# daultanigaurav/AI-BASED-FRAME-INTERPOLATION

Measured on AMD Instinct MI355X. Metric: interpolated frames/sec at 1080p, higher is better.
Workload: dtype bf16

## Files before the change

ai_based_frame_interpolation_amd/csrc/conv3x3_mfma.hip.h:

```cpp
#pragma once
#include <hip/hip_runtime.h>
#include <stdint.h>
#include <type_traits>

namespace fiunet {

typedef __attribute__((ext_vector_type(4))) float f32x4;
typedef __attribute__((ext_vector_type(8))) __bf16 bf16x8;
typedef __attribute__((ext_vector_type(8))) _Float16 f16x8;

enum SrcMode { SRC_DIRECT = 0, SRC_POOL = 1 , SRC_CONCAT_UP = 2,
               SRC_STEM = 3 ,
               SRC_DIRECT_X2 = 4,
               SRC_STEM_X2 = 5 };
constexpr bool src_is_stem(int mode) { return mode == SRC_STEM || mode == SRC_STEM_X2; }
constexpr bool src_is_x2(int mode) { return mode == SRC_DIRECT_X2 || mode == SRC_STEM_X2; }

__device__ __forceinline__ size_t blk_off(int plane, int y, int x, int H, int W)
{
    return (((size_t)plane * H + y) * W + x) * 64;
}

struct ConvArgs {
    const void* src0;
// ... 159 lines not shown
                                              float ly)
{
    constexpr int NE = Elem<T>::NE;
    float fa[NE], fb[NE], fc[NE], fd[NE], r[NE];
    chunk_unpack<T>(a, fa); chunk_unpack<T>(b, fb); chunk_unpack<T>(c, fc); chunk_unpack<T>(d, fd);
#pragma unroll
    for (int i = 0; i < NE; ++i) {
        const float top = fmaf(lx, fb[i], __fmul_rn(hx, fa[i]));
        const float bot = fmaf(lx, fd[i], __fmul_rn(hx, fc[i]));
        r[i] = fmaf(ly, bot, __fmul_rn(hy, top));
    }
    return chunk_pack<T>(r);
}

template <typename T>
__device__ __forceinline__ void chunk_hlerp(const uint4& a, const uint4& b, float hx, float lx, float* h)
{
    constexpr int NE = Elem<T>::NE;
    float fa[NE], fb[NE];
    chunk_unpack<T>(a, fa); chunk_unpack<T>(b, fb);
#pragma unroll
    for (int i = 0; i < NE; ++i) h[i] = fmaf(lx, fb[i], __fmul_rn(hx, fa[i]));
}
template <typename T>
__device__ __forceinline__ uint4 chunk_vlerp(const float* top, const float* bot, float hy, float ly)
{
    constexpr int NE = Elem<T>::NE;
    float r[NE];
#pragma unroll
    for (int i = 0; i < NE; ++i) r[i] = fmaf(ly, bot[i], __fmul_rn(hy, top[i]));
    return chunk_pack<T>(r);
}


__device__ __forceinline__ uint4 ldg16(const char* p) { return *reinterpret_cast<const uint4*>(p); }

__device__ __forceinline__ float preprocess_u8_value(unsigned char u)
{
    const float x = (float)u, r = 1.0f / 255.0f;
    const float q0 = __fmul_rn(x, r);
    const float q = fmaf(fmaf(-q0, 255.0f, x), r, q0);
    return __fsub_rn(__fmul_rn(2.0f, q), 1.0f);
}
__device__ __forceinline__ unsigned char postprocess_u8_value(float x)
{
    float v = __fdiv_rn(__fadd_rn(x, 1.0f), 2.0f);
    v = fminf(fmaxf(v, 0.0f), 1.0f);
    return (unsigned char)(int)__fmul_rn(v, 255.0f);
}

__device__ __forceinline__ float stem_dither(int y, int x)
{
    const unsigned a = (unsigned)(x ^ y) & 7u, b = (unsigned)y & 7u;
    const unsigned m = ((a & 1u) << 5) | ((b & 1u) << 4) | ((a & 2u) << 2) | ((b & 2u) << 1) | ((a & 4u) >> 1) | ((b & 4u) >> 2);
    return ((float)m + 0.5f) * (1.0f / 64.0f) - 0.5f;
}

struct UpAxis {
    int i0, i1;
    float h, l;
    bool ok;
};
__device__ __forceinline__ UpAxis up_axis(int c, int off, int pad, int lowNg, float scale, int lowOff,
                                          int lowN)
{
    UpAxis u;
    int cu = c + off - pad;
    u.ok = (cu >= 0) & (cu < 2 * lowNg);
    cu = min(max(cu, 0), 2 * lowNg - 1);
    const float f = scale * (float)cu;
    const int g0 = (int)f;
    const int g1 = g0 < lowNg - 1 ? g0 + 1 : g0;
    u.l = f - (float)g0;
    u.h = 1.0f - u.l;
    u.i0 = min(max(g0 - lowOff, 0), lowN - 1);
    u.i1 = min(max(g1 - lowOff, 0), lowN - 1);
    return u;
}
__device__ __forceinline__ UpAxis up_axis_y(const ConvArgs& a, int y)
{
    return up_axis(y, a.upOffY, a.padT, a.lowHg, a.sy, a.lowOffY, a.lowH);
}
__device__ __forceinline__ UpAxis up_axis_x(const ConvArgs& a, int x)
{
    return up_axis(x, 0, a.padL, a.lowW, a.sx, 0, a.lowW);
}
struct UpCoord {
    int y0, y1, x0, x1;
    float hy, ly, hx, lx;
    bool ok;
};
__device__ __forceinline__ UpCoord up_coord(const ConvArgs& a, int y, int x)
{
    const UpAxis v = up_axis_y(a, y), h = up_axis_x(a, x);
    UpCoord u;
    u.y0 = v.i0; u.y1 = v.i1; u.hy = v.h; u.ly = v.l;
    u.x0 = h.i0; u.x1 = h.i1; u.hx = h.h; u.lx = h.l;
    u.ok = v.ok & h.ok;
    return u;
}

template <typename T, int MODE>
__device__ __forceinline__ uint4 gather_chunk(const ConvArgs& a, int b, int y, int x, int plane,
                                              int ch)
{
    constexpr int PL = Elem<T>::PL;
    bool ok = (y >= 0) & (y < a.H) & (x >= 0) & (x < a.W);
    y = min(max(y, 0), a.H - 1);
    x = min(max(x, 0), a.W - 1);
    const int p0 = a.C0 / PL;
    uint4 v;
    if (MODE == SRC_DIRECT || plane < p0) {
        const char* p = (const char*)a.src0 + (size_t)b * a.H * a.W * a.C0 * sizeof(T) +
                        blk_off(plane, y, x, a.H, a.W) + ch * 16;
        v = ldg16(p);
    } else {
        const UpCoord u = up_coord(a, y, x);
        ok = ok & u.ok;
        const char* base = (const char*)a.src1 + (size_t)b * a.lowH * a.lowW * a.C1 * sizeof(T) + ch * 16;
        const int q = plane - p0;
        const uint4 v00 = ldg16(base + blk_off(q, u.y0, u.x0, a.lowH, a.lowW));
        const uint4 v01 = ldg16(base + blk_off(q, u.y0, u.x1, a.lowH, a.lowW));
        const uint4 v10 = ldg16(base + blk_off(q, u.y1, u.x0, a.lowH, a.lowW));
        const uint4 v11 = ldg16(base + blk_off(q, u.y1, u.x1, a.lowH, a.lowW));
        v = chunk_bilerp<T>(v00, v01, v10, v11, u.hx, u.lx, u.hy, u.ly);
    }
    return ok ? v : make_uint4(0u, 0u, 0u, 0u);
}

__device__ __forceinline__ void glds16(const char* gsrc, unsigned lds_wave_base)
{
    unsigned keep;
    asm volatile("s_mov_b32 %0, m0\n\ts_mov_b32 m0, %2\n\ts_nop 0\n\t"
                 "global_load_lds_dwordx4 %1, off\n\ts_mov_b32 m0, %0"
                 : "=&s"(keep)
                 : "v"(gsrc), "s"(lds_wave_base)
                 : "memory");
}
__device__ __forceinline__ void glds16s(const char* sbase, unsigned voff, unsigned lds_wave_base)
{
    unsigned keep;
    asm volatile("s_mov_b32 %0, m0\n\ts_mov_b32 m0, %3\n\ts_nop 0\n\t"
                 "global_load_lds_dwordx4 %1, %2\n\ts_mov_b32 m0, %0"
                 : "=&s"(keep)
                 : "v"(voff), "s"(sbase), "s"(lds_wave_base)
                 : "memory");
}
__device__ __forceinline__ void lds_dma_wait_all() { asm volatile("s_waitcnt vmcnt(0)" ::: "memory"); }
__device__ __forceinline__ unsigned lds_addr_of(const char* p)
{
    return (unsigned)(uintptr_t)(__attribute__((address_space(3))) const char*)p;
}

__device__ __forceinline__ int swz(int row) { return ((row >> 2) & 1) << 1; }

template <typename T>
__device__ __forceinline__ void mma_chunk(f32x4& acc, const uint4& wa, const uint4& xb);
template <>
__device__ __forceinline__ void mma_chunk<__bf16>(f32x4& acc, const uint4& wa, const uint4& xb)
{
    acc = __builtin_amdgcn_mfma_f32_16x16x32_bf16(__builtin_bit_cast(bf16x8, wa),
                                                  __builtin_bit_cast(bf16x8, xb), acc, 0, 0, 0);
}
template <>
__device__ __forceinline__ void mma_chunk<_Float16>(f32x4& acc, const uint4& wa, const uint4& xb)
{
    acc = __builtin_amdgcn_mfma_f32_16x16x32_f16(__builtin_bit_cast(f16x8, wa),
                                                 __builtin_bit_cast(f16x8, xb), acc, 0, 0, 0);
}
template <>
__device__ __forceinline__ void mma_chunk<float>(f32x4& acc, const uint4& wa, const uint4& xb)
{
    acc = __builtin_amdgcn_mfma_f32_16x16x4f32(__uint_as_float(wa.x), __uint_as_float(xb.x), acc, 0, 0, 0);
    acc = __builtin_amdgcn_mfma_f32_16x16x4f32(__uint_as_float(wa.y), __uint_as_float(xb.y), acc, 0, 0, 0);
    acc = __builtin_amdgcn_mfma_f32_16x16x4f32(__uint_as_float(wa.z), __uint_as_float(xb.z), acc, 0, 0, 0);
    acc = __builtin_amdgcn_mfma_f32_16x16x4f32(__uint_as_float(wa.w), __uint_as_float(xb.w), acc, 0, 0, 0);
}

enum Epilogue { EPI_PLAIN = 0, EPI_HEAD = 1 , EPI_POOL = 2, EPI_HEAD3 = 3 ,
                EPI_SPLITK = 4  };
constexpr bool epi_is_splitk(int epi) { return epi == EPI_SPLITK; }

__device__ __forceinline__ unsigned dpp_swap_pairs(unsigned v)
{
    return (unsigned)__builtin_amdgcn_update_dpp(0, (int)v, 0xB1, 0xF, 0xF, true);
}

constexpr int up_segments(int rows, int ncol)
{
    int best = 1, best_cost = 1 << 30;
    for (int n = 1; n <= 6; ++n) {
        const int passes = (n * ncol + 255) / 256, segr = (rows + n - 1) / n;
        const int cost = passes * (segr * 4 + 3);
        if (cost < best_cost) { best_cost = cost; best = n; }
    }
    return best;
}

template <int BN, int TH, int TW, int MODE> struct ConvTile {
    static constexpr int TWP = ((TW + 2 + 7) / 8) * 8;
    static constexpr int THP = TH + 2;
    static constexpr int IN_BYTES = THP * TWP * 64;
    static constexpr int W_BYTES = 3 * BN * 64;
    static constexpr int LRH = (TH + 1) / 2 + 3, LRW = (TW + 1) / 2 + 3, LRP = ((LRW + 3) / 4) * 4;
    static constexpr int LR_PIECES = (LRH * LRP + 15) / 16;
    static constexpr int SPARE_BYTES =
        (MODE == SRC_CONCAT_UP && LR_PIECES * 1024 > W_BYTES) ? LR_PIECES * 1024 - W_BYTES : 0;
    static constexpr int W_STRIDE = W_BYTES + SPARE_BYTES;
    static constexpr int PATCH_W = TW + 4, PATCH_H = TH + 4, PATCH_PITCH = 2 * PATCH_W;
    static_assert(!src_is_stem(MODE) || (2 * PATCH_PITCH) % 32 == 16, "patch pitch: lane groups 0/1 must not share banks");
    static constexpr int PATCH_OFF = IN_BYTES + 2 * W_BYTES + SPARE_BYTES;
    static constexpr int PATCH_TAIL_OFF = (TW + 2) * 64;
    static constexpr int PATCH_TAIL = 2 * PATCH_W * 4;
    static_assert(!src_is_stem(MODE) || PATCH_TAIL_OFF + PATCH_TAIL <= TWP * 64, "bias operand must fit the row-pitch filler");
    static constexpr int PATCH_BYTES = src_is_stem(MODE) ? PATCH_H * PATCH_PITCH * 4 : 0;
    static constexpr int TAB_OFF = PATCH_OFF + ((PATCH_BYTES + 15) / 16) * 16;
    static constexpr int TAB_BYTES = MODE == SRC_CONCAT_UP ? ((THP + TW + 2) * 16 + 255) / 256 * 256 : 0;
    static constexpr int STEMW_OFF = TAB_OFF + TAB_BYTES;
    static constexpr int STEMW_BYTES = src_is_stem(MODE) ? 4096 : 0;
    static constexpr int LDS_BYTES = STEMW_OFF + STEMW_BYTES;
    static_assert(LDS_BYTES <= 80 * 1024, "two workgroups must fit in the CU's 160 KiB of LDS");
    static_assert(!src_is_stem(MODE) || LDS_BYTES <= 63 * 1280, "fused-stem kernel: stay below 64 LDS granules");
};

constexpr int conv_wave_frags(int BN, int TH, int TW) { return TH * TW / 16 / (4 / (BN / 64)); }
constexpr int conv_occupancy(int BN, int TH, int TW, int lds_bytes = 0)
{
    return conv_wave_frags(BN, TH, TW) == 4 && lds_bytes * 3 <= 160 * 1024 ? 3 : 2;
}


__device__ __forceinline__ int conv_block_remap()
{
    const int nblk = gridDim.x, bid = blockIdx.x;
    const int q = nblk >> 3, r = nblk & 7, xcd = bid & 7;
    return (xcd < r ? xcd * (q + 1) : r * (q + 1) + (xcd - r) * q) + (bid >> 3);
}

struct ConvTileId { int ct, b, ty, tx; };
__device__ __forceinline__ ConvTileId conv_tile_decode(const ConvArgs& a, int t)
{
    ConvTileId d;
    d.ct = t % a.nct; t /= a.nct;
    d.tx = t % a.tilesX; t /= a.tilesX;
    d.ty = t % a.tilesY;
    d.b = t / a.tilesY;
    return d;
}

template <typename T> __device__ __forceinline__ int conv_cout_ofs(int m, int lc)
{
    return sizeof(T) == 2 ? (m >> 1) * 32 + lc * 8 + (m & 1) * 4 : m * 16 + lc * 4;
}

template <typename T, int BN, int TH, int TW, int EPI>
__device__ __forceinline__ void conv_acc_init(const ConvArgs& a, f32x4 (&acc)[4][conv_wave_frags(BN, TH, TW)],
                                              int ct, int wc, int lc)
{
    constexpr int NF = conv_wave_frags(BN, TH, TW);
#pragma unroll
    for (int m = 0; m < 4; ++m) {
        f32x4 v = f32x4{0.f, 0.f, 0.f, 0.f};
        if constexpr (!epi_is_splitk(EPI)) {
            const float4 sh = *reinterpret_cast<const float4*>(a.shift + ct * BN + wc * 64 + conv_cout_ofs<T>(m, lc));
            v = f32x4{sh.x, sh.y, sh.z, sh.w};
        }
#pragma unroll
        for (int n = 0; n < NF; ++n) acc[m][n] = v;
    }
}

__device__ __forceinline__ unsigned relu_pk_bf16(unsigned p) { return pk_max_i16(p, 0u); }
__device__ __forceinline__ void relu_fma(float& sum, float x, float lo, float w)
{
    float t;
    asm("v_max_f32 %1, %3, %2\n\tv_fmac_f32 %0, %1, %4" : "+v"(sum), "=&v"(t) : "v"(x), "v"(lo), "v"(w));
}

template <typename T, int BN, int TH, int TW, int EPI, bool X2 = false>
__device__ __forceinline__ void conv_epilogue(const ConvArgs& a, f32x4 (&acc)[4][conv_wave_frags(BN, TH, TW)],
                                              int b, int y0, int x0, int ct, int split, int wc, int wp,
                                              int l15, int lc)
{
    constexpr int PL = Elem<T>::PL;
    constexpr int FR = TW / 16;
    constexpr int NF = conv_wave_frags(BN, TH, TW);
    constexpr int ROWS_W = NF / FR;
    constexpr int HNC = EPI == EPI_HEAD ? 1 : (EPI == EPI_HEAD3 ? 3 : 0);
    const int aH = a.H, aW = a.W;
    constexpr bool PERM = sizeof(T) == 2;
    const int wbase_c = ct * BN + wc * 64;
    if constexpr (epi_is_splitk(EPI)) {
        const int tile = (((b * a.tilesY) + y0 / TH) * a.tilesX + x0 / TW) * a.nct + ct;
        const int ntile = a.B * a.tilesY * a.tilesX * a.nct;
        const int wave = wp * (BN / 64) + wc;
        float4* o = reinterpret_cast<float4*>(a.kslab) + ((((size_t)split * ntile + tile) * 4 + wave) * (4 * NF)) * 64 + (lc * 16 + l15);
#pragma unroll
        for (int m = 0; m < 4; ++m)
#pragma unroll
            for (int n = 0; n < NF; ++n)
                o[(m * NF + n) * 64] = make_float4(acc[m][n][0], acc[m][n][1], acc[m][n][2], acc[m][n][3]);
        return;
    }
    float hw[HNC > 0 ? HNC : 1][4][4];
#pragma unroll
    for (int c = 0; c < HNC; ++c)
#pragma unroll
        for (int m = 0; m < 4; ++m) {
            const float4 v = *reinterpret_cast<const float4*>(a.head_w + c * 64 + conv_cout_ofs<T>(m, lc));
            hw[c][m][0] = v.x; hw[c][m][1] = v.y; hw[c][m][2] = v.z; hw[c][m][3] = v.w;
        }
    const size_t plane_stride = (size_t)aH * aW * 64;
    const int plane0 = wbase_c / PL;
    const int rec_byte = lc * 16;
    char* const out_img = a.dst ? (char*)a.dst + (size_t)b * plane_stride * (a.Cout / PL) +
                                  (size_t)plane0 * plane_stride + rec_byte : nullptr;
    const int pH = aH >> 1, pW = aW >> 1;
    const size_t pplane_stride = (size_t)pH * pW * 64;
    char* const pool_img = EPI == EPI_POOL ? (char*)a.pool_dst + (size_t)b * pplane_stride * (a.Cout / PL) +
                                             (size_t)plane0 * pplane_stride + rec_byte : nullptr;
    if constexpr (HNC > 0) {
        static_assert(HNC == 0 || NF == 8 || NF == 4, "head reduction is written for 8 or 4 fragments per wave");
        const float floor_v = a.relu ? 0.f : -__builtin_inff();
        float hb[HNC];
#pragma unroll
        for (int c = 0; c < HNC; ++c) hb[c] = a.head_b[c];
        const int nb = ((lc & 1) ? 4 : 0) + ((lc & 2) ? 2 : 0);
#pragma unroll
        for (int c = 0; c < HNC; ++c) {
            float hs[NF];
#pragma unroll
            for (int n = 0; n < NF; ++n) {
                float sum = 0.f;
#pragma unroll
                for (int m = 0; m < 4; ++m)
#pragma unroll
                    for (int j = 0; j < 4; ++j) relu_fma(sum, acc[m][n][j], floor_v, hw[c][m][j]);
                hs[n] = sum;
            }
            if constexpr (NF == 4) {
                float full[NF];
#pragma unroll
                for (int n = 0; n < NF; ++n) {
                    const float p = hs[n] + __shfl_xor(hs[n], 16);
                    full[n] = p + __shfl_xor(p, 32);
                }
                const float mine = lc == 0 ? full[0] : (lc == 1 ? full[1] : (lc == 2 ? full[2] : full[3]));
                const int n = lc;
                const int y = y0 + wp * ROWS_W + n / FR;
                const int x = x0 + (n % FR) * 16 + l15;
                if (y < aH && x < aW) {
                    const size_t o = (size_t)b * a.head_img_stride + ((size_t)c * aH + y) * aW + x;
                    if (a.head_out_u8) a.head_out_u8[o] = postprocess_u8_value(mine + hb[c]);
                    else a.head_out[o] = mine + hb[c];
                }
            } else {
                float t[4], u[2];
#pragma unroll
                for (int i = 0; i < 4; ++i) {
                    const auto r = __builtin_amdgcn_permlane16_swap(__float_as_uint(hs[i]), __float_as_uint(hs[(i + 4) % NF]), false, false);
                    t[i] = __uint_as_float(r[0]) + __uint_as_float(r[1]);
                }
#pragma unroll
                for (int j = 0; j < 2; ++j) {
                    const auto r = __builtin_amdgcn_permlane32_swap(__float_as_uint(t[j]), __float_as_uint(t[j + 2]), false, false);
                    u[j] = __uint_as_float(r[0]) + __uint_as_float(r[1]);
                }
#pragma unroll
                for (int j = 0; j < 2; ++j) {
                    const int n = nb + j;
                    const int y = y0 + wp * ROWS_W + n / FR;
                    const int x = x0 + (n % FR) * 16 + l15;
                    if (y < aH && x < aW) {
// ... 102 lines not shown
                const uint4 t = pk[0][g], u = pk[1][g];
                const unsigned c0 = pk_max_i16(t.x, u.x), c1 = pk_max_i16(t.y, u.y);
                const unsigned c2 = pk_max_i16(t.z, u.z), c3 = pk_max_i16(t.w, u.w);
                const uint4 m = make_uint4(pk_max_i16(c0, dpp_swap_pairs(c0)), pk_max_i16(c1, dpp_swap_pairs(c1)),
                                           pk_max_i16(c2, dpp_swap_pairs(c2)), pk_max_i16(c3, dpp_swap_pairs(c3)));
                if (okp) *reinterpret_cast<uint4*>(o + g * pplane_stride) = m;
            }
        }
        return;
    }
#pragma unroll
    for (int n = 0; n < NF; ++n) {
        const int y = y0 + wp * ROWS_W + n / FR;
        const int x = x0 + (n % FR) * 16 + l15;
        const bool ok = (y < aH) && (x < aW);
        if (ok && out_img) {
            char* o = out_img + (size_t)(y * aW + x) * 64;
            if constexpr (PERM) {
#pragma unroll
                for (int g = 0; g < 2; ++g) {
                    uint4 pk = make_uint4(pack2<T>(acc[2 * g][n][0], acc[2 * g][n][1]),
                                          pack2<T>(acc[2 * g][n][2], acc[2 * g][n][3]),
                                          pack2<T>(acc[2 * g + 1][n][0], acc[2 * g + 1][n][1]),
                                          pack2<T>(acc[2 * g + 1][n][2], acc[2 * g + 1][n][3]));
                    if (a.relu) pk = make_uint4(relu_pk_bf16(pk.x), relu_pk_bf16(pk.y), relu_pk_bf16(pk.z), relu_pk_bf16(pk.w));
                    *reinterpret_cast<uint4*>(o + g * plane_stride) = pk;
                }
            } else {
#pragma unroll
                for (int m = 0; m < 4; ++m) {
                    float4 v = make_float4(acc[m][n][0], acc[m][n][1], acc[m][n][2], acc[m][n][3]);
                    if (a.relu) v = make_float4(fmaxf(v.x, 0.f), fmaxf(v.y, 0.f), fmaxf(v.z, 0.f), fmaxf(v.w, 0.f));
                    *reinterpret_cast<float4*>(o + m * plane_stride) = v;
                }
            }
        }
    }
    if (EPI == EPI_POOL) {
#pragma unroll
        for (int n = 0; n < NF; ++n) {
            if (((n / FR) & 1) != 0) continue;
            const int y = y0 + wp * ROWS_W + n / FR;
            const int x = x0 + (n % FR) * 16 + l15;
            const int py = y >> 1, px = x >> 1;
            const bool okp = (py < pH) && (px < pW) && ((l15 & 1) == 0);
            char* o = pool_img + (size_t)(min(py, pH - 1) * pW + min(px, pW - 1)) * 64;
            if constexpr (!PERM) {
#pragma unroll
                for (int m = 0; m < 4; ++m) {
                    float r[4];
#pragma unroll
                    for (int j = 0; j < 4; ++j) {
                        const float cm = fmaxf(acc[m][n][j], acc[m][n + FR][j]);
                        r[j] = fmaxf(cm, __uint_as_float(dpp_swap_pairs(__float_as_uint(cm))));
                        if (a.relu) r[j] = fmaxf(r[j], 0.f);
                    }
                    if (okp) *reinterpret_cast<float4*>(o + m * pplane_stride) = make_float4(r[0], r[1], r[2], r[3]);
                }
            } else {
#pragma unroll
                for (int g = 0; g < 2; ++g) {
                    unsigned r[4];
#pragma unroll
                    for (int h = 0; h < 2; ++h) {
                        const int m = 2 * g + h;
                        const unsigned a0 = pk_max_i16(pack2_pk<T>(acc[m][n][0], acc[m][n][1]),
                                                       pack2_pk<T>(acc[m][n + FR][0], acc[m][n + FR][1]));
                        const unsigned a1 = pk_max_i16(pack2_pk<T>(acc[m][n][2], acc[m][n][3]),
                                                       pack2_pk<T>(acc[m][n + FR][2], acc[m][n + FR][3]));
                        r[2 * h] = pk_max_i16(a0, dpp_swap_pairs(a0));
                        r[2 * h + 1] = pk_max_i16(a1, dpp_swap_pairs(a1));
                        if (a.relu) { r[2 * h] = relu_pk_bf16(r[2 * h]); r[2 * h + 1] = relu_pk_bf16(r[2 * h + 1]); }
                    }
                    if (okp) *reinterpret_cast<uint4*>(o + g * pplane_stride) = make_uint4(r[0], r[1], r[2], r[3]);
                }
            }
        }
    }
}

template <typename T, int BN, int TH, int TW, int MODE, int EPI>
__global__ __launch_bounds__(256, conv_occupancy(BN, TH, TW, ConvTile<BN, TH, TW, MODE>::LDS_BYTES)) void conv3x3_mfma_kernel(const ConvArgs a)
{
    using Tile = ConvTile<BN, TH, TW, MODE>;
    constexpr int PL = Elem<T>::PL;
    constexpr int TWP = Tile::TWP, THP = Tile::THP;
    constexpr int WAVES_C = BN / 64, WAVES_P = 4 / WAVES_C;
    constexpr int FR = TW / 16;
    constexpr int NF = conv_wave_frags(BN, TH, TW);
    constexpr int ROWS_W = NF / FR;
    static_assert(NF == 8 || NF == 4, "wave tile must be 64 couts x 128 or 64 pixels");
    static_assert(TH == ROWS_W * WAVES_P && ROWS_W * FR == NF, "tile does not split over the waves");
    static_assert(EPI != EPI_POOL || ROWS_W % 2 == 0, "pooled epilogue: a wave owns whole row pairs");
    static_assert(Tile::LDS_BYTES * conv_occupancy(BN, TH, TW, Tile::LDS_BYTES) <= 160 * 1024, "LDS per CU");
    constexpr int HNC = EPI == EPI_HEAD ? 1 : (EPI == EPI_HEAD3 ? 3 : 0);
    static_assert(HNC == 0 || BN == 64, "fused head needs all 64 couts in one wave");
    static_assert(MODE == SRC_DIRECT || MODE == SRC_CONCAT_UP || MODE == SRC_STEM || MODE == SRC_DIRECT_X2 ||
                  MODE == SRC_STEM_X2, "pooling is fused into the producer");
    constexpr bool X2 = src_is_x2(MODE);
    constexpr bool STEM = src_is_stem(MODE);
    constexpr bool DIRECT = MODE == SRC_DIRECT || MODE == SRC_DIRECT_X2;
    static_assert(!X2 || std::is_same_v<T, __bf16>, "two-piece operands are bf16");
    static_assert(!STEM || (sizeof(T) == 2 && BN == 64), "fused stem: 2-byte output (bf16 / fp16), 64 couts");

    extern __shared__ __attribute__((aligned(16))) char smem[];
    char* const lds_in = smem;
    char* const lds_w = smem + Tile::IN_BYTES;
    const unsigned lds_in_addr = lds_addr_of(lds_in);
    const unsigned lds_w_addr = lds_addr_of(lds_w);

    int lid = conv_block_remap();
    const int ksplit = epi_is_splitk(EPI) ? a.ksplit : 1;
    const int split = lid % ksplit;
    lid /= ksplit;
    const ConvTileId id = conv_tile_decode(a, lid);
    const int ct = id.ct, b = id.b;
    const int y0 = id.ty * TH, x0 = id.tx * TW;

    const int tid = threadIdx.x;
    const int lane = tid & 63, wave = __builtin_amdgcn_readfirstlane(tid >> 6);
    const int l15 = lane & 15, lc = lane >> 4;
    const int wc = wave % WAVES_C, wp = wave / WAVES_C;

#ifdef FIUNET_STAMP
    unsigned long long st_sum[16] = {0, 0, 0, 0, 0, 0, 0, 0, 0, 0, 0, 0, 0, 0, 0, 0};
    unsigned long long st_t0 = __builtin_amdgcn_s_memtime(), st_prev = st_t0;
#ifdef FIUNET_STAMP_PROLOG
    unsigned long long st_pprev = st_t0;
#define PSTAMP(slot) do { __builtin_amdgcn_sched_barrier(0); const unsigned long long t_ = __builtin_amdgcn_s_memtime(); \
                          st_sum[slot] += t_ - st_pprev; st_pprev = t_; __builtin_amdgcn_sched_barrier(0); } while (0)
#else
#define PSTAMP(slot) do {} while (0)
#endif
#define STAMP(slot) do { const unsigned long long t_ = __builtin_amdgcn_s_memtime(); \
                         st_sum[slot] += t_ - st_prev; st_prev = t_; } while (0)
#define STAMP_UP(slot) STAMP(slot)
#else
#define STAMP(slot) do {} while (0)
#define STAMP_UP(slot) do {} while (0)
#define PSTAMP(slot) do {} while (0)
#endif
    f32x4 acc[4][NF];
    conv_acc_init<T, BN, TH, TW, EPI>(a, acc, ct, wc, lc);
#ifdef FIUNET_STAMP_PROLOG
    asm volatile("" :: "v"(acc[3][NF - 1][3]), "v"(acc[0][0][0]));
#endif
    PSTAMP(9);

    const int a_off = (wc * 64 + l15) * 64 + ((lc ^ swz(l15)) << 4);
    int b_off[3];
#pragma unroll
    for (int kx = 0; kx < 3; ++kx)
        b_off[kx] = (wp * ROWS_W * TWP + kx + l15) * 64 + ((lc ^ swz(kx + l15)) << 4);

    const int nplanes_real = (a.C0 + a.C1) / PL;
    const int nplanes_all = X2 ? 3 * nplanes_real : nplanes_real;
    const int p0 = a.C0 / PL;
    const int pbeg = split * nplanes_all / ksplit, pend = (split + 1) * nplanes_all / ksplit;
    const int nsteps = (pend - pbeg) * 3;
    const char* wbase = (const char*)a.wgt + (size_t)ct * BN * 64;

    constexpr int NW = Tile::W_BYTES / 1024 / 4;
    static_assert(BN % 16 == 0, "a weight piece must not straddle two taps");
    const unsigned w_lane_off = (unsigned)((lane >> 2) * 64 + (((lane & 3) ^ swz(lane >> 2)) << 4));
    auto issue_w = [&](int step) __attribute__((always_inline)) {
        const int lp = step / 3, kx = step - lp * 3;
        int pl = pbeg + lp;
        if constexpr (X2) {
            const int real = pl / 3;
            pl = pl - real * 3 == 1 ? nplanes_real + real : real;
        }
        const char* wsrc = wbase + ((size_t)(pl * 9 + kx * 3) * a.Cout) * 64;
        const unsigned dst = __builtin_amdgcn_readfirstlane(
            lds_w_addr + (unsigned)((step & 1) * Tile::W_STRIDE + wave * NW * 1024));
#pragma unroll
        for (int j = 0; j < NW; ++j) {
            const int r0 = (wave * NW + j) * 16, tap = r0 / BN;
            glds16s(wsrc + (size_t)(tap * (a.Cout - BN) + r0) * 64, w_lane_off, dst + j * 1024);
        }
    };
#ifndef FIUNET_DIAG_FREE_PROLOGUE
    issue_w(0);
#endif
#ifdef FIUNET_DIAG_NO_WSTREAM
    if (nsteps > 1) issue_w(1);
#endif
    PSTAMP(10);

    constexpr int NPIECE = THP * TWP / 16;
    static_assert(THP * TWP % 16 == 0, "in-tile must be a whole number of 1-KiB pieces");
    const int aH = a.H, aW = a.W;
    const char* const dma_src = (const char*)a.src0 + (size_t)b * a.H * a.W * a.C0 * sizeof(T) * (X2 ? 2 : 1);
    const char* const dma_src1 = DIRECT && a.C1 > 0
                                     ? (const char*)a.src1 + (size_t)b * a.H * a.W * a.C1 * sizeof(T) * (X2 ? 2 : 1) : nullptr;
    constexpr bool HOIST = (MODE == SRC_DIRECT && BN == 128 && EPI == EPI_PLAIN) ||
                           (NF == 4 && DIRECT);
    constexpr bool ROLL = sizeof(T) == 2 && FR == 2 && (!epi_is_splitk(EPI) || NF == 4);
    constexpr int NPW = (NPIECE + 3) / 4;
    unsigned in_off[HOIST ? NPW : 1];
    const unsigned plane_bytes = (unsigned)(aH * aW) * 64u;
    unsigned pm_lin0 = 0, pm_valid = 0, pm_wrap = 0;
    static_assert(NPW <= 32, "one mask bit per piece of a wave");
    constexpr int PM_DY = 64 / TWP, PM_DX = 64 % TWP;
    const unsigned pm_dlin = (unsigned)(PM_DY * aW + PM_DX) * 64u, pm_dwrap = (unsigned)(aW - TWP) * 64u;
    if constexpr (!STEM) {
        const int row0 = wave * 16 + (lane >> 2);
        int py = row0 / TWP, px = row0 - py * TWP;
        int y = y0 - 1 + py, x = x0 - 1 + px;
        pm_lin0 = (unsigned)(y * aW + x) * 64u + (((lane & 3) ^ swz(row0)) << 4);
        unsigned lin = pm_lin0;
#pragma unroll
        for (int jj = 0; jj < NPW; ++jj) {
            const bool ok = (px < TW + 2) & ((unsigned)y < (unsigned)aH) & ((unsigned)x < (unsigned)aW);
            if constexpr (HOIST) in_off[jj] = ok ? lin : ~0u;
            pm_valid |= (ok ? 1u : 0u) << jj;
            px += PM_DX; x += PM_DX; y += PM_DY;
            lin += pm_dlin;
            if (px >= TWP) { px -= TWP; x -= TWP; y += 1; pm_wrap |= 1u << jj; lin += pm_dwrap; }
        }
    }
    auto for_pieces = [&](auto&& f) __attribute__((always_inline)) {
        if constexpr (HOIST) {
#pragma unroll
            for (int jj = 0; jj < NPW; ++jj) {
                const int j = wave + 4 * jj;
                if (j < NPIECE) f(j, in_off[jj] != ~0u, in_off[jj]);
            }
        } else {
            unsigned lin = pm_lin0, valid = pm_valid, wrap = pm_wrap;
            asm volatile("" : "+v"(lin), "+v"(valid), "+v"(wrap));
#pragma unroll
            for (int jj = 0; jj < NPW; ++jj) {
                const int j = wave + 4 * jj;
                if (j < NPIECE) f(j, ((valid >> jj) & 1u) != 0u, lin);
                lin += pm_dlin + (((wrap >> jj) & 1u) ? pm_dwrap : 0u);
            }
        }
    };
    if constexpr (!STEM) {
        for_pieces([&](int j, bool ok, unsigned) __attribute__((always_inline)) {
            if (!ok) *reinterpret_cast<uint4*>(lds_in + j * 1024 + lane * 16) = make_uint4(0u, 0u, 0u, 0u);
        });
    }
    auto gather_plane_dma = [&](int plane) __attribute__((always_inline)) {
        const char* base;
        if constexpr (X2) {
            const int real = plane / 3, lo = plane - real * 3 == 2;
            base = real >= p0 ? dma_src1 + (size_t)(real - p0 + (lo ? nplanes_real - p0 : 0)) * plane_bytes
                              : dma_src + (size_t)(real + (lo ? p0 : 0)) * plane_bytes;
        } else {
            base = (MODE == SRC_DIRECT && plane >= p0) ? dma_src1 + (size_t)(plane - p0) * plane_bytes
                                                       : dma_src + (size_t)plane * plane_bytes;
        }
        for_pieces([&](int j, bool ok, unsigned off) __attribute__((always_inline)) {
            if (ok) glds16s(base, off, __builtin_amdgcn_readfirstlane(lds_in_addr + (unsigned)j * 1024u));
        });
    };

    constexpr int UP_NCOL = (TW + 2) * 4;
    constexpr int UP_NMAIN = UP_NCOL / 64;
    constexpr int UP_NTC = UP_NCOL - UP_NMAIN * 64;
    constexpr int UP_WPG = 4 / UP_NMAIN;
    constexpr int UP_SEGR = (THP + UP_WPG - 1) / UP_WPG;
    constexpr int UP_NTAIL = UP_NTC * THP;
    constexpr int UP_TAILW = (UP_NTAIL + 3) / 4;
    static_assert(MODE != SRC_CONCAT_UP || (UP_NMAIN >= 1 && UP_NMAIN <= 2), "interpolation work split");
    int lr_y = 0, lr_x = 0;
    char* const ytab = smem + Tile::TAB_OFF;
    char* const xtab = ytab + THP * 16;
    uint4 yrow = make_uint4(0u, 0u, 0u, 0u);
    if constexpr (MODE == SRC_CONCAT_UP) {
        const UpCoord u = up_coord(a, y0 - 1, x0 - 1);
        lr_y = u.y0; lr_x = u.x0;
        {
            const int y = y0 - 1 + min(lane, THP - 1);
            const UpAxis uy = up_axis_y(a, min(max(y, 0), a.H - 1));
            const bool ok = uy.ok & (y >= 0) & (y < a.H);
            yrow = make_uint4(ok ? (unsigned)((uy.i0 - lr_y) * (Tile::LRP * 64)) : 0x80000000u,
                              (unsigned)((uy.i1 - lr_y) * (Tile::LRP * 64)), __float_as_uint(uy.h),
                              __float_as_uint(uy.l));
            if (tid < THP) *reinterpret_cast<uint4*>(ytab + tid * 16) = yrow;
        }
        if (tid >= 64 && tid < 64 + TW + 2) {
            const int px = tid - 64, x = x0 - 1 + px;
            const UpAxis ux = up_axis_x(a, min(max(x, 0), a.W - 1));
            const bool ok = ux.ok & (x >= 0) & (x < a.W);
            *reinterpret_cast<uint4*>(xtab + px * 16) =
                make_uint4(ok ? (unsigned)((ux.i0 - lr_x) * 64) : 0x80000000u, (unsigned)((ux.i1 - lr_x) * 64),
                           __float_as_uint(ux.h), __float_as_uint(ux.l));
        }
    }
    auto gather_plane_up = [&](int plane, int idle_slot) __attribute__((always_inline)) {
        constexpr int LRP = Tile::LRP, LRH = Tile::LRH;
        const int stg_off = idle_slot == 0 ? 0 : Tile::W_BYTES;
        const char* const lsrc = (const char*)a.src1 + (size_t)b * a.lowH * a.lowW * a.C1 * sizeof(T) +
                                 (size_t)(plane - p0) * a.lowH * a.lowW * 64;
        int opq = 0;
        asm volatile("" : "+s"(opq));
        int l4 = (lane & 3) << 4;
        asm volatile("" : "+v"(l4));
#pragma unroll 1
        for (int j = wave; j < Tile::LR_PIECES; j += 4) {
            const int row = j * 16 + (lane >> 2) + opq;
            const int r = row / LRP, c = row - r * LRP;
            const int gy = min(lr_y + min(r, LRH - 1), a.lowH - 1), gx = min(lr_x + c, a.lowW - 1);
            const char* src = lsrc + ((unsigned)(gy * a.lowW + gx) * 64u + (unsigned)l4);
            glds16(src, __builtin_amdgcn_readfirstlane(lds_w_addr + (unsigned)(stg_off + j * 1024)));
        }
        lds_dma_wait_all();
        __syncthreads();
        STAMP_UP(6);
        const char* const stg = lds_w + stg_off;
        constexpr int NE = Elem<T>::NE;
        {
            const int grp = UP_NMAIN == 1 ? 0 : (wave & 1), seg = UP_NMAIN == 1 ? wave : (wave >> 1);
            const int col = grp * 64 + lane, px = col >> 2, ch = col & 3;
            const uint4 xt = *reinterpret_cast<const uint4*>(xtab + px * 16);
            const bool okx = (int)xt.x >= 0;
            const char* const s0 = stg + (okx ? (int)xt.x : 0) + ch * 16;
            const char* const s1 = stg + (okx ? (int)xt.y : 0) + ch * 16;
            const float hx = okx ? __uint_as_float(xt.z) : 0.f, lx = okx ? __uint_as_float(xt.w) : 0.f;
            float h0[NE], h1[NE];
#pragma unroll
            for (int i = 0; i < NE; ++i) h0[i] = h1[i] = 0.f;
            int c0 = -1, c1 = -1;
            const int rbeg = seg * UP_SEGR, rend = min(THP, rbeg + UP_SEGR);
#pragma unroll 1
            for (int py = rbeg; py < rend; ++py) {
                const uint4 yt = make_uint4((unsigned)__builtin_amdgcn_readlane((int)yrow.x, py),
                                            (unsigned)__builtin_amdgcn_readlane((int)yrow.y, py),
                                            (unsigned)__builtin_amdgcn_readlane((int)yrow.z, py),
                                            (unsigned)__builtin_amdgcn_readlane((int)yrow.w, py));
                const int o0 = (int)yt.x, o1 = (int)yt.y;
                uint4 v = make_uint4(0u, 0u, 0u, 0u);
                if (o0 >= 0) {
                    if (o0 != c0) {
                        if (o0 == c1) {
#pragma unroll
                            for (int i = 0; i < NE; ++i) h0[i] = h1[i];
                        } else {
                            chunk_hlerp<T>(*reinterpret_cast<const uint4*>(s0 + o0),
                                           *reinterpret_cast<const uint4*>(s1 + o0), hx, lx, h0);
                        }
                        c0 = o0;
                    }
                    if (o1 != c1) {
                        if (o1 == c0) {
#pragma unroll
                            for (int i = 0; i < NE; ++i) h1[i] = h0[i];
                        } else {
                            chunk_hlerp<T>(*reinterpret_cast<const uint4*>(s0 + o1),
                                           *reinterpret_cast<const uint4*>(s1 + o1), hx, lx, h1);
                        }
                        c1 = o1;
                    }
                    v = chunk_vlerp<T>(h0, h1, __uint_as_float(yt.z), __uint_as_float(yt.w));
                }
                const int row = py * TWP + px;
                *reinterpret_cast<uint4*>(lds_in + row * 64 + ((ch ^ swz(row)) << 4)) = v;
            }
        }
        for (int k = lane; k < UP_TAILW; k += 64) {
            const int e = wave * UP_TAILW + k;
            if (e < UP_NTAIL) {
                const int py = e / UP_NTC, col = UP_NMAIN * 64 + (e - py * UP_NTC), px = col >> 2, ch = col & 3;
                const uint4 xt = *reinterpret_cast<const uint4*>(xtab + px * 16);
                const uint4 yt = *reinterpret_cast<const uint4*>(ytab + py * 16);
                const bool ok = ((int)xt.x >= 0) & ((int)yt.x >= 0);
                const char* const q0 = stg + (ok ? (int)xt.x : 0) + ch * 16;
                const char* const q1 = stg + (ok ? (int)xt.y : 0) + ch * 16;
                const int o0 = ok ? (int)yt.x : 0, o1 = ok ? (int)yt.y : 0;
                uint4 v = chunk_bilerp<T>(*reinterpret_cast<const uint4*>(q0 + o0), *reinterpret_cast<const uint4*>(q1 + o0),
                                          *reinterpret_cast<const uint4*>(q0 + o1), *reinterpret_cast<const uint4*>(q1 + o1),
                                          __uint_as_float(xt.z), __uint_as_float(xt.w), __uint_as_float(yt.z),
                                          __uint_as_float(yt.w));
                if (!ok) v = make_uint4(0u, 0u, 0u, 0u);
                const int row = py * TWP + px;
                *reinterpret_cast<uint4*>(lds_in + row * 64 + ((ch ^ swz(row)) << 4)) = v;
            }
        }
        STAMP_UP(7);
    };

    constexpr int NIN = THP * (TW + 2);
    char* const patch = smem + Tile::PATCH_OFF;
    constexpr int PW = Tile::PATCH_W, PH = Tile::PATCH_H, PP = Tile::PATCH_PITCH;
    auto stage_patch = [&]() __attribute__((always_inline)) {
        if constexpr (STEM) {
            unsigned* const pd = reinterpret_cast<unsigned*>(patch);
            constexpr int NP = PH * PW;
            constexpr int NB = (NP + 255) / 256;
            float v0[NB], v1[NB];
            unsigned okm = 0;
            size_t at[NB];
#pragma unroll
            for (int k = 0; k < NB; ++k) {
                const int r = tid + k * 256;
                const int py = r / PW, px = r - py * PW;
                const int y = y0 - 2 + py, x = x0 - 2 + px;
                const bool ok = (r < NP) & (y >= 0) & (y < aH) & (x >= 0) & (x < aW);
                okm |= (ok ? 1u : 0u) << k;
                at[k] = ((size_t)b * aH + min(max(y, 0), aH - 1)) * aW + min(max(x, 0), aW - 1);
            }
            if (a.u1) {
                unsigned char q0[NB], q1[NB];
#pragma unroll
                for (int k = 0; k < NB; ++k) { q0[k] = a.u1[at[k]]; q1[k] = a.u2[at[k]]; }
#pragma unroll
                for (int k = 0; k < NB; ++k) { v0[k] = preprocess_u8_value(q0[k]); v1[k] = preprocess_u8_value(q1[k]); }
            } else {
#pragma unroll
                for (int k = 0; k < NB; ++k) { v0[k] = a.f1[at[k]]; v1[k] = a.f2[at[k]]; }
            }
#pragma unroll
            for (int k = 0; k < NB; ++k) {
                const int r = tid + k * 256;
                const int py = r / PW, px = r - py * PW;
                const float d = a.dither * stem_dither(y0 - 2 + py, x0 - 2 + px);
                const bool ok = (okm >> k) & 1u;
                v0[k] = ok ? v0[k] + d : 0.f;
                v1[k] = ok ? v1[k] - d : 0.f;
            }
#pragma unroll
            for (int k = 0; k < NB; ++k) {
                const int r = tid + k * 256;
                const int py = r / PW, px = r - py * PW;
                const unsigned hi = pack_bf16x2_pk(v0[k], v1[k]);
                const unsigned lo = pack_bf16x2_pk(v0[k] - __uint_as_float(hi << 16), v1[k] - __uint_as_float(hi & 0xffff0000u));
                if (r < NP) {
                    pd[py * PP + px] = hi;
                    pd[py * PP + px + PW] = lo;
                }
            }
            if (tid < 2 * PW) reinterpret_cast<unsigned*>(smem + Tile::PATCH_TAIL_OFF)[tid] = tid < PW ? 0x00003f80u : 0u;
        }
    };
    struct StemW { uint4 wh[2], wl[2]; };
    StemW stem_w0;
    auto stem_park = [&](int plane) __attribute__((always_inline)) {
        if constexpr (STEM && X2)
            glds16s((const char*)a.stem_w + (wave >> 1) * 4096 + (2 * plane + (wave & 1)) * 1024, (unsigned)lane * 16u,
                    __builtin_amdgcn_readfirstlane(lds_in_addr + (unsigned)(Tile::STEMW_OFF + wave * 1024)));
        else if constexpr (STEM)
            glds16((const char*)a.stem_w + (wave >> 1) * 4096 + (2 * plane + (wave & 1)) * 1024 + lane * 16,
                   __builtin_amdgcn_readfirstlane(lds_in_addr + (unsigned)(Tile::STEMW_OFF + wave * 1024)));
    };
    auto stem_load = [&](StemW& w) __attribute__((always_inline)) {
        if constexpr (STEM) {
            int lane_ofs = l15 * 64 + lc * 16;
            asm volatile("" : "+v"(lane_ofs));
#pragma unroll
            for (int h = 0; h < 2; ++h) {
                w.wh[h] = ldg16((const char*)a.stem_w + h * 1024 + lane_ofs);
                w.wl[h] = ldg16((const char*)a.stem_w + 4096 + h * 1024 + lane_ofs);
            }
            stem_park(X2 ? 0 : 1);
        }
    };
    auto stem_parked = [&](StemW& w) __attribute__((always_inline)) {
        if constexpr (STEM) {
            const char* const base = smem + Tile::STEMW_OFF + l15 * 64 + lc * 16;
#pragma unroll
            for (int h = 0; h < 2; ++h) {
                w.wh[h] = *reinterpret_cast<const uint4*>(base + h * 1024);
                w.wl[h] = *reinterpret_cast<const uint4*>(base + 2048 + h * 1024);
            }
        }
    };
    auto gather_plane_stem = [&](const StemW& w, bool lo_piece = false) __attribute__((always_inline)) {
        if constexpr (STEM) {
            constexpr int TAIL_IDX = (Tile::PATCH_TAIL_OFF - Tile::PATCH_OFF) / 4;
            const unsigned* const ph32 = reinterpret_cast<const unsigned*>(patch);
            const unsigned* const pl32 = ph32 + PW;
            struct Frag { uint4 bh, bl; int dst; };
            constexpr int DY = 64 / (TW + 2), DX = 64 % (TW + 2);
            const int py0 = (wave * 16 + l15) / (TW + 2);
            int px = wave * 16 + l15 - py0 * (TW + 2);
            int e = lc < 3 ? py0 * PP + px + (lc == 0 ? 0 : (lc == 1 ? 2 * PP : PP)) : TAIL_IDX;
            const int e_step = lc < 3 ? DY * PP + DX : 0, e_wrap = lc < 3 ? PP - (TW + 2) : 0;
            int dst = py0 * TWP + px;
            auto fetch = [&](Frag& f) __attribute__((always_inline)) {
                f.bh = make_uint4(ph32[e], ph32[e + 1], ph32[e + 2], ph32[e + 3]);
                f.bl = make_uint4(pl32[e], pl32[e + 1], pl32[e + 2], pl32[e + 3]);
                f.dst = dst;
                px += DX;
                const bool wrap = px >= TW + 2;
                px -= wrap ? TW + 2 : 0;
                e += e_step + (wrap ? e_wrap : 0);
                dst += DY * TWP + DX + (wrap ? TWP - (TW + 2) : 0);
            };
            auto compute = [&](const Frag& f) __attribute__((always_inline)) {
                f32x4 s4[2];
#pragma unroll
                for (int h = 0; h < 2; ++h) s4[h] = f32x4{0.f, 0.f, 0.f, 0.f};
#pragma unroll
                for (int h = 0; h < 2; ++h) mma_chunk<__bf16>(s4[h], w.wl[h], f.bh);
#pragma unroll
                for (int h = 0; h < 2; ++h) mma_chunk<__bf16>(s4[h], w.wh[h], f.bl);
#pragma unroll
                for (int h = 0; h < 2; ++h) mma_chunk<__bf16>(s4[h], w.wh[h], f.bh);
                const int row = f.dst;
                uint4 pk = make_uint4(relu_pk_bf16(pack2_pk<T>(s4[0][0], s4[0][1])),
                                      relu_pk_bf16(pack2_pk<T>(s4[0][2], s4[0][3])),
                                      relu_pk_bf16(pack2_pk<T>(s4[1][0], s4[1][1])),
                                      relu_pk_bf16(pack2_pk<T>(s4[1][2], s4[1][3])));
                if constexpr (X2) {
                    if (lo_piece) {
                        auto lo2 = [](float v0, float v1, unsigned hi) __attribute__((always_inline)) {
                            return pack_bf16x2_pk(fmaxf(v0, 0.f) - __uint_as_float(hi << 16),
                                                  fmaxf(v1, 0.f) - __uint_as_float(hi & 0xffff0000u));
                        };
                        pk = make_uint4(lo2(s4[0][0], s4[0][1], pk.x), lo2(s4[0][2], s4[0][3], pk.y),
                                        lo2(s4[1][0], s4[1][1], pk.z), lo2(s4[1][2], s4[1][3], pk.w));
                    }
                }
                if (row < THP * TWP) *reinterpret_cast<uint4*>(lds_in + ((row * 64 + lc * 16) ^ ((row & 4) << 3))) = pk;
            };
            constexpr int NQ = (NIN + 15) / 16;
            Frag fa, fb;
            fetch(fa);
#pragma unroll 1
            for (int q = wave; q < NQ; q += 8) {
                fetch(fb);
                compute(fa);
                fetch(fa);
                if (q + 4 < NQ) compute(fb);
            }
            if ((y0 == 0) | (x0 == 0) | (y0 + TH >= aH) | (x0 + TW >= aW)) {
                __syncthreads();
                for (int i = tid; i < THP * (TW + 2) * 4; i += 256) {
                    const int q = i >> 2, ch = i & 3;
                    const int qy = q / (TW + 2), qx = q - qy * (TW + 2);
                    const bool in = ((unsigned)(y0 - 1 + qy) < (unsigned)aH) & ((unsigned)(x0 - 1 + qx) < (unsigned)aW);
                    const int row = qy * TWP + qx;
                    if (!in) *reinterpret_cast<uint4*>(lds_in + row * 64 + ((ch ^ swz(row)) << 4)) = make_uint4(0u, 0u, 0u, 0u);
                }
            }
        }
    };
    auto gather_plane = [&](int plane, int idle_slot, bool first) __attribute__((always_inline)) {
        if constexpr (STEM && X2) {
            if (first) {
                gather_plane_stem(stem_w0, false);
            } else {
                StemW w;
                stem_parked(w);
                gather_plane_stem(w, plane == 2 || plane == 5);
            }
        } else if constexpr (STEM) {
            if (first) {
                gather_plane_stem(stem_w0);
            } else {
                StemW w1;
                stem_parked(w1);
                gather_plane_stem(w1);
            }
        }
        else if (DIRECT || plane < p0) gather_plane_dma(plane);
        else gather_plane_up(plane, idle_slot);
    };

    PSTAMP(11);
    if constexpr (STEM) {
        stem_load(stem_w0);
        stage_patch();
        __syncthreads();
        PSTAMP(12);
    }
#ifdef FIUNET_DIAG_FREE_PROLOGUE
    if constexpr (STEM || MODE == SRC_CONCAT_UP) gather_plane(pbeg, 1, true);
#else
    gather_plane(pbeg, 1, true);
#endif
    PSTAMP(13);
    lds_dma_wait_all();
    PSTAMP(14);
    __syncthreads();
    PSTAMP(15);
    STAMP(1);
#ifdef FIUNET_CLOCK
    const unsigned long long ck_t0 = __builtin_amdgcn_s_memtime(), ck_r0 = __builtin_amdgcn_s_memrealtime();
#endif

    int step = 0;
    int vj = X2 ? pbeg % 3 : 0;
    for (int plane = pbeg; plane < pend; ++plane) {
        const bool gather_next = plane + 1 < pend && !(X2 && vj == 0);
        if constexpr (X2) vj = vj == 2 ? 0 : vj + 1;
#pragma unroll
        for (int kx = 0; kx < 3; ++kx, ++step) {
#ifndef FIUNET_DIAG_NO_WSTREAM
            if (step + 1 < nsteps) issue_w(step + 1);
#endif
            const char* wcur = lds_w + (step & 1) * Tile::W_STRIDE + a_off;
            constexpr bool EARLY_OK = ROLL && DIRECT;
            bool early = false;
            if constexpr (EARLY_OK)
                early = kx == 2 && gather_next && (DIRECT || plane + 1 < p0);
            if constexpr (ROLL) {
                uint4 xb[ROWS_W + 2][FR];
                auto load_row = [&](int i) __attribute__((always_inline)) {
#pragma unroll
                    for (int f = 0; f < FR; ++f)
                        xb[i][f] = *reinterpret_cast<const uint4*>(lds_in + b_off[kx] + (i * TWP + f * 16) * 64);
                };
#pragma unroll
                for (int i = 0; i < ROWS_W; ++i) load_row(i);
#pragma unroll
                for (int ky = 0; ky < 3; ++ky) {
                    uint4 wa[4];
#pragma unroll
                    for (int m = 0; m < 4; ++m)
                        wa[m] = *reinterpret_cast<const uint4*>(wcur + (ky * BN + m * 16) * 64);
                    if (ky < 2) load_row(ROWS_W + ky);
                    if (ky == 1 && early) {
                        __syncthreads();
                        gather_plane(plane + 1, step & 1, false);
                    }
#pragma unroll
                    for (int m = 0; m < 4; ++m)
#pragma unroll
                        for (int n = 0; n < NF; ++n) mma_chunk<T>(acc[m][n], wa[m], xb[n / FR + ky][n % FR]);
                }
            } else {
#pragma unroll
                for (int ky = 0; ky < 3; ++ky) {
                    asm volatile("" ::: "memory");
                    uint4 wa[4], xb[NF];
#pragma unroll
                    for (int m = 0; m < 4; ++m)
                        wa[m] = *reinterpret_cast<const uint4*>(wcur + (ky * BN + m * 16) * 64);
#pragma unroll
                    for (int n = 0; n < NF; ++n)
                        xb[n] = *reinterpret_cast<const uint4*>(
                            lds_in + b_off[kx] + (((n / FR) + ky) * TWP + (n % FR) * 16) * 64);
#pragma unroll
                    for (int m = 0; m < 4; ++m)
#pragma unroll
                        for (int n = 0; n < NF; ++n) mma_chunk<T>(acc[m][n], wa[m], xb[n]);
                }
            }
#ifdef FIUNET_STAMP
            asm volatile("" :: "v"(acc[3][NF - 1][3]));
            __builtin_amdgcn_sched_barrier(0);
#endif
            STAMP(2);
            if (kx == 2 && gather_next && !early) {
                __syncthreads();
                gather_plane(plane + 1, step & 1, false);
                lds_dma_wait_all();
                __syncthreads();
                if constexpr (STEM && X2) { if (plane + 1 == 2) stem_park(1); }
                STAMP(4);
            } else {
                lds_dma_wait_all();
                __syncthreads();
                STAMP(3);
            }
        }
    }

#ifdef FIUNET_CLOCK
    {
        asm volatile("" :: "v"(acc[3][NF - 1][3]));
        __builtin_amdgcn_sched_barrier(0);
        const unsigned long long ck_t1 = __builtin_amdgcn_s_memtime(), ck_r1 = __builtin_amdgcn_s_memrealtime();
        const unsigned st_idx = blockIdx.x * 4u + (unsigned)wave;
        if (a.stamp && lane == 0 && st_idx < a.stamp_cap) {
            unsigned long long* rec = a.stamp + (size_t)st_idx * 16;
            rec[0] = ck_t1 - ck_t0;
            rec[1] = ck_r1 - ck_r0;
            rec[8] = 1ull;
        }
    }
#endif
    conv_epilogue<T, BN, TH, TW, EPI, X2>(a, acc, b, y0, x0, ct, split, wc, wp, l15, lc);
#ifdef FIUNET_STAMP
    STAMP(5);
    st_sum[0] = st_prev - st_t0;
    const unsigned st_idx = blockIdx.x * 4u + (unsigned)wave;
    if (a.stamp && lane == 0 && st_idx < a.stamp_cap) {
        unsigned long long* rec = a.stamp + (size_t)st_idx * 16;
#pragma unroll
        for (int k = 0; k < 16; ++k) rec[k] = k == 8 ? 1ull : st_sum[k];
    }
#endif
}

template <typename T, int BN, int TH, int TW, int EPI, bool X2>
__global__ __launch_bounds__(64) void splitk_finalize_tile_kernel(const ConvArgs a)
{
    static_assert(EPI == EPI_PLAIN || EPI == EPI_POOL, "a fused head is never K-split");
    constexpr int WAVES_C = BN / 64;
    constexpr int NF = conv_wave_frags(BN, TH, TW);
    int t = blockIdx.x >> 2;
    const int tile = t;
    const int ct = t % a.nct; t /= a.nct;
    const int tx = t % a.tilesX; t /= a.tilesX;
    const int ty = t % a.tilesY;
    const int b = t / a.tilesY;
    const int lane = threadIdx.x & 63, wave = blockIdx.x & 3;
    const int l15 = lane & 15, lc = lane >> 4;
    const int wc = wave % WAVES_C, wp = wave / WAVES_C;
    const int ntile = a.B * a.tilesY * a.tilesX * a.nct;
    f32x4 acc[4][NF];
#pragma unroll
    for (int m = 0; m < 4; ++m)
#pragma unroll
        for (int n = 0; n < NF; ++n) acc[m][n] = f32x4{0.f, 0.f, 0.f, 0.f};
    const float4* p = reinterpret_cast<const float4*>(a.kslab) + (((size_t)tile * 4 + wave) * (4 * NF)) * 64 + lane;
    const size_t slice = (size_t)ntile * 4 * (4 * NF) * 64;
    const int ks = a.ksplit;
#pragma unroll
    for (int m = 0; m < 4; ++m) {
        const float4* pm = p + (size_t)m * NF * 64;
        constexpr int CH = NF == 8 ? 2 : 4;
        for (int s0 = 0; s0 < ks; s0 += CH, pm += CH * slice) {
            float4 q[CH][NF];
#pragma unroll
            for (int j = 0; j < CH; ++j)
                if (s0 + j < ks) {
#pragma unroll
                    for (int n = 0; n < NF; ++n) q[j][n] = pm[j * slice + n * 64];
                }
#pragma unroll
            for (int j = 0; j < CH; ++j)
                if (s0 + j < ks) {
#pragma unroll
                    for (int n = 0; n < NF; ++n) {
                        acc[m][n][0] += q[j][n].x; acc[m][n][1] += q[j][n].y; acc[m][n][2] += q[j][n].z; acc[m][n][3] += q[j][n].w;
                    }
                }
        }
    }
#pragma unroll
    for (int m = 0; m < 4; ++m) {
        const float4 sh = *reinterpret_cast<const float4*>(a.shift + ct * BN + wc * 64 + conv_cout_ofs<T>(m, lc));
#pragma unroll
        for (int n = 0; n < NF; ++n) {
            acc[m][n][0] += sh.x; acc[m][n][1] += sh.y; acc[m][n][2] += sh.z; acc[m][n][3] += sh.w;
        }
    }
    conv_epilogue<T, BN, TH, TW, EPI, X2>(a, acc, b, ty * TH, tx * TW, ct, 0, wc, wp, l15, lc);
}

}
```

Baseline: 527.6.

## Cut VGPR pressure in concat-up conv and enable early next-plane DMA gather

For the concat-up source mode, the per-piece mask state is parked in LDS, the lane id is recomputed on demand, and the B-operand offset is rebuilt from one base with an XOR swizzle. Together these shorten live ranges of values that were held across the main loop. The change also turns on the early next-plane gather for concat-up, issuing a DMA gather in the middle of the ky loop so it overlaps the MFMA work. The trade is extra LDS space and a few extra LDS reads and ALU ops, plus the risk of getting the swizzle or sync ordering wrong.

```diff
diff --git a/ai_based_frame_interpolation_amd/csrc/conv3x3_mfma.hip.h b/ai_based_frame_interpolation_amd/csrc/conv3x3_mfma.hip.h
--- a/ai_based_frame_interpolation_amd/csrc/conv3x3_mfma.hip.h
+++ b/ai_based_frame_interpolation_amd/csrc/conv3x3_mfma.hip.h
@@ -335,6 +335,12 @@
     return (unsigned)(uintptr_t)(__attribute__((address_space(3))) const char*)p;
 }
 
+__device__ __forceinline__ int lane_id_fresh()
+{
+    int l;
+    asm volatile("v_mbcnt_lo_u32_b32 %0, -1, 0\n\tv_mbcnt_hi_u32_b32 %0, -1, %0" : "=v"(l));
+    return l;
+}
 __device__ __forceinline__ int swz(int row) { return ((row >> 2) & 1) << 1; }
 
 template <typename T>
@@ -401,7 +407,9 @@
     static constexpr int TAB_BYTES = MODE == SRC_CONCAT_UP ? ((THP + TW + 2) * 16 + 255) / 256 * 256 : 0;
     static constexpr int STEMW_OFF = TAB_OFF + TAB_BYTES;
     static constexpr int STEMW_BYTES = src_is_stem(MODE) ? 4096 : 0;
-    static constexpr int LDS_BYTES = STEMW_OFF + STEMW_BYTES;
+    static constexpr int PM_OFF = STEMW_OFF + STEMW_BYTES;
+    static constexpr int PM_BYTES = MODE == SRC_CONCAT_UP && TW == 32 && TH * TW / 16 / (4 / (BN / 64)) == 8 ? 3 * 256 * 4 : 0;
+    static constexpr int LDS_BYTES = PM_OFF + PM_BYTES;
     static_assert(LDS_BYTES <= 80 * 1024, "two workgroups must fit in the CU's 160 KiB of LDS");
     static_assert(!src_is_stem(MODE) || LDS_BYTES <= 63 * 1280, "fused-stem kernel: stay below 64 LDS granules");
 };
@@ -810,6 +818,9 @@
 #pragma unroll
     for (int kx = 0; kx < 3; ++kx)
         b_off[kx] = (wp * ROWS_W * TWP + kx + l15) * 64 + ((lc ^ swz(kx + l15)) << 4);
+    constexpr bool DIET = Tile::PM_BYTES > 0 && sizeof(T) == 2;
+    static_assert(!DIET || (ROWS_W * TWP) % 8 == 0, "the swizzle phase must not depend on the wave");
+    const int b_base = (wp * ROWS_W * TWP + l15) * 64 + (lc << 4);
 
     const int nplanes_real = (a.C0 + a.C1) / PL;
     const int nplanes_all = X2 ? 3 * nplanes_real : nplanes_real;
@@ -858,6 +869,7 @@
     unsigned in_off[HOIST ? NPW : 1];
     const unsigned plane_bytes = (unsigned)(aH * aW) * 64u;
     unsigned pm_lin0 = 0, pm_valid = 0, pm_wrap = 0;
+    constexpr bool PM_LDS = DIET;
     static_assert(NPW <= 32, "one mask bit per piece of a wave");
     constexpr int PM_DY = 64 / TWP, PM_DX = 64 % TWP;
     const unsigned pm_dlin = (unsigned)(PM_DY * aW + PM_DX) * 64u, pm_dwrap = (unsigned)(aW - TWP) * 64u;
@@ -876,6 +888,10 @@
             lin += pm_dlin;
             if (px >= TWP) { px -= TWP; x -= TWP; y += 1; pm_wrap |= 1u << jj; lin += pm_dwrap; }
         }
+        if constexpr (PM_LDS) {
+            unsigned* const pm = reinterpret_cast<unsigned*>(smem + Tile::PM_OFF) + tid;
+            pm[0] = pm_lin0; pm[256] = pm_valid; pm[512] = pm_wrap;
+        }
     }
     auto for_pieces = [&](auto&& f) __attribute__((always_inline)) {
         if constexpr (HOIST) {
@@ -886,6 +902,10 @@
             }
         } else {
             unsigned lin = pm_lin0, valid = pm_valid, wrap = pm_wrap;
+            if constexpr (PM_LDS) {
+                const unsigned* const pm = reinterpret_cast<const unsigned*>(smem + Tile::PM_OFF) + wave * 64 + lane_id_fresh();
+                lin = pm[0]; valid = pm[256]; wrap = pm[512];
+            }
             asm volatile("" : "+v"(lin), "+v"(valid), "+v"(wrap));
 #pragma unroll
             for (int jj = 0; jj < NPW; ++jj) {
@@ -926,18 +946,16 @@
     int lr_y = 0, lr_x = 0;
     char* const ytab = smem + Tile::TAB_OFF;
     char* const xtab = ytab + THP * 16;
-    uint4 yrow = make_uint4(0u, 0u, 0u, 0u);
     if constexpr (MODE == SRC_CONCAT_UP) {
         const UpCoord u = up_coord(a, y0 - 1, x0 - 1);
-        lr_y = u.y0; lr_x = u.x0;
-        {
-            const int y = y0 - 1 + min(lane, THP - 1);
+        lr_y = __builtin_amdgcn_readfirstlane(u.y0); lr_x = __builtin_amdgcn_readfirstlane(u.x0);
+        if (tid < THP) {
+            const int y = y0 - 1 + tid;
             const UpAxis uy = up_axis_y(a, min(max(y, 0), a.H - 1));
             const bool ok = uy.ok & (y >= 0) & (y < a.H);
-            yrow = make_uint4(ok ? (unsigned)((uy.i0 - lr_y) * (Tile::LRP * 64)) : 0x80000000u,
-                              (unsigned)((uy.i1 - lr_y) * (Tile::LRP * 64)), __float_as_uint(uy.h),
-                              __float_as_uint(uy.l));
-            if (tid < THP) *reinterpret_cast<uint4*>(ytab + tid * 16) = yrow;
+            *reinterpret_cast<uint4*>(ytab + tid * 16) =
+                make_uint4(ok ? (unsigned)((uy.i0 - lr_y) * (Tile::LRP * 64)) : 0x80000000u,
+                           (unsigned)((uy.i1 - lr_y) * (Tile::LRP * 64)), __float_as_uint(uy.h), __float_as_uint(uy.l));
         }
         if (tid >= 64 && tid < 64 + TW + 2) {
             const int px = tid - 64, x = x0 - 1 + px;
@@ -955,11 +973,11 @@
                                  (size_t)(plane - p0) * a.lowH * a.lowW * 64;
         int opq = 0;
         asm volatile("" : "+s"(opq));
-        int l4 = (lane & 3) << 4;
-        asm volatile("" : "+v"(l4));
+        const int ln = lane_id_fresh();
+        const int l4 = (ln & 3) << 4;
 #pragma unroll 1
         for (int j = wave; j < Tile::LR_PIECES; j += 4) {
-            const int row = j * 16 + (lane >> 2) + opq;
+            const int row = j * 16 + (ln >> 2) + opq;
             const int r = row / LRP, c = row - r * LRP;
             const int gy = min(lr_y + min(r, LRH - 1), a.lowH - 1), gx = min(lr_x + c, a.lowW - 1);
             const char* src = lsrc + ((unsigned)(gy * a.lowW + gx) * 64u + (unsigned)l4);
@@ -970,9 +988,10 @@
         STAMP_UP(6);
         const char* const stg = lds_w + stg_off;
         constexpr int NE = Elem<T>::NE;
+        const uint4 yrow = *reinterpret_cast<const uint4*>(ytab + min(ln, THP - 1) * 16);
         {
             const int grp = UP_NMAIN == 1 ? 0 : (wave & 1), seg = UP_NMAIN == 1 ? wave : (wave >> 1);
-            const int col = grp * 64 + lane, px = col >> 2, ch = col & 3;
+            const int col = grp * 64 + ln, px = col >> 2, ch = col & 3;
             const uint4 xt = *reinterpret_cast<const uint4*>(xtab + px * 16);
             const bool okx = (int)xt.x >= 0;
             const char* const s0 = stg + (okx ? (int)xt.x : 0) + ch * 16;
@@ -1018,7 +1037,7 @@
                 *reinterpret_cast<uint4*>(lds_in + row * 64 + ((ch ^ swz(row)) << 4)) = v;
             }
         }
-        for (int k = lane; k < UP_TAILW; k += 64) {
+        for (int k = ln; k < UP_TAILW; k += 64) {
             const int e = wave * UP_TAILW + k;
             if (e < UP_NTAIL) {
                 const int py = e / UP_NTC, col = UP_NMAIN * 64 + (e - py * UP_NTC), px = col >> 2, ch = col & 3;
@@ -1251,16 +1270,27 @@
             if (step + 1 < nsteps) issue_w(step + 1);
 #endif
             const char* wcur = lds_w + (step & 1) * Tile::W_STRIDE + a_off;
+#ifdef FIUNET_DIAG_FREE_SKIP_BOUNDARY
             constexpr bool EARLY_OK = ROLL && DIRECT;
+#else
+            constexpr bool EARLY_OK = ROLL && (DIRECT || MODE == SRC_CONCAT_UP);
+#endif
             bool early = false;
             if constexpr (EARLY_OK)
                 early = kx == 2 && gather_next && (DIRECT || plane + 1 < p0);
+            int b_cur = b_off[kx];
+            if constexpr (DIET) {
+                int t = b_base;
+                asm volatile("" : "+v"(t));
+                t += kx * 64;
+                b_cur = t ^ ((t >> 3) & 32);
+            }
             if constexpr (ROLL) {
                 uint4 xb[ROWS_W + 2][FR];
                 auto load_row = [&](int i) __attribute__((always_inline)) {
 #pragma unroll
                     for (int f = 0; f < FR; ++f)
-                        xb[i][f] = *reinterpret_cast<const uint4*>(lds_in + b_off[kx] + (i * TWP + f * 16) * 64);
+                        xb[i][f] = *reinterpret_cast<const uint4*>(lds_in + b_cur + (i * TWP + f * 16) * 64);
                 };
 #pragma unroll
                 for (int i = 0; i < ROWS_W; ++i) load_row(i);
@@ -1273,7 +1303,8 @@
                     if (ky < 2) load_row(ROWS_W + ky);
                     if (ky == 1 && early) {
                         __syncthreads();
-                        gather_plane(plane + 1, step & 1, false);
+                        if constexpr (MODE == SRC_CONCAT_UP) gather_plane_dma(plane + 1);
+                        else gather_plane(plane + 1, step & 1, false);
                     }
 #pragma unroll
                     for (int m = 0; m < 4; ++m)
@@ -1291,7 +1322,7 @@
 #pragma unroll
                     for (int n = 0; n < NF; ++n)
                         xb[n] = *reinterpret_cast<const uint4*>(
-                            lds_in + b_off[kx] + (((n / FR) + ky) * TWP + (n % FR) * 16) * 64);
+                            lds_in + b_cur + (((n / FR) + ky) * TWP + (n % FR) * 16) * 64);
 #pragma unroll
                     for (int m = 0; m < 4; ++m)
 #pragma unroll
@@ -1303,7 +1334,12 @@
             __builtin_amdgcn_sched_barrier(0);
 #endif
             STAMP(2);
-            if (kx == 2 && gather_next && !early) {
+#ifdef FIUNET_DIAG_FREE_SKIP_BOUNDARY
+            const bool free_boundary = MODE == SRC_CONCAT_UP && plane + 1 < p0;
+#else
+            constexpr bool free_boundary = false;
+#endif
+            if (kx == 2 && gather_next && !early && !free_boundary) {
                 __syncthreads();
                 gather_plane(plane + 1, step & 1, false);
                 lds_dma_wait_all();
@@ -1332,7 +1368,12 @@
         }
     }
 #endif
-    conv_epilogue<T, BN, TH, TW, EPI, X2>(a, acc, b, y0, x0, ct, split, wc, wp, l15, lc);
+    if constexpr (MODE == SRC_CONCAT_UP) {
+        const int ln = lane_id_fresh();
+        conv_epilogue<T, BN, TH, TW, EPI, X2>(a, acc, b, y0, x0, ct, split, wc, wp, ln & 15, ln >> 4);
+    } else {
+        conv_epilogue<T, BN, TH, TW, EPI, X2>(a, acc, b, y0, x0, ct, split, wc, wp, l15, lc);
+    }
 #ifdef FIUNET_STAMP
     STAMP(5);
     st_sum[0] = st_prev - st_t0;
```

New measurement: 531.5 (median of 2 runs). Within noise of the previous version (+0.7%).
